# algbio/founderblockgraphs

Measured on AMD Instinct MI355X. Metric: MSA columns segmented/sec, higher is better.
Workload: dtype u32

## Files before the change

founderblockgraphs_amd/csrc/ctx.hip:

```cpp
#include "fbg_internal.h"
#include <chrono>
#include <stdarg.h>
#include <stdio.h>
#include <ctype.h>
#include <string.h>
#include <algorithm>
#include <atomic>
#include <thread>
#include <vector>

static std::string g_global_err;

int fbg_fail(fbg_ctx *ctx, int code, const char *fmt, ...)
{
    char buf[1024];
    va_list ap;
    va_start(ap, fmt);
    vsnprintf(buf, sizeof(buf), fmt, ap);
    va_end(ap);
    if (ctx) ctx->err = buf; else g_global_err = buf;
    return code;
}

int fbg_reserve(fbg_ctx *ctx, DevBuf &b, size_t bytes, std::vector<DevBuf *> *owner, bool accounted)
// ... 166 lines not shown
    {"pure_scan", &FbgOptions::pure_scan},
    {"gapped_rank", &FbgOptions::gapped_rank},
    {"part_tricks_off", &FbgOptions::part_tricks_off},
    {"msd_sample_bins", &FbgOptions::msd_sample_bins},
    {"msd_min_force", &FbgOptions::msd_min_force},
    {"msd_probe", &FbgOptions::msd_probe},
    {"msd_xcd", &FbgOptions::msd_xcd},
    {"rank_no_lean", &FbgOptions::rank_no_lean},
    {"no_stream_upload", &FbgOptions::no_stream_upload},
    {"span_scan", &FbgOptions::span_scan},
    {"span_key_flags", &FbgOptions::span_key_flags},
    {"span_slow_split", &FbgOptions::span_slow_split},
    {"poison", &FbgOptions::poison},
    {"dpw_matrix", &FbgOptions::dpw_matrix},
    {"dp_chain1", &FbgOptions::dp_chain1},
    {"msd_ext", &FbgOptions::msd_ext},
    {"rows_wave", &FbgOptions::rows_wave},
    {"pairs_in_scan", &FbgOptions::pairs_in_scan},
    {"runs_wave_min", &FbgOptions::runs_wave_min},
    {"wave_list_cap", &FbgOptions::wave_list_cap},
    {"cand_local_sort", &FbgOptions::cand_local_sort},
    {"cand_lds_cap", &FbgOptions::cand_lds_cap},
    {"cand_sort_check", &FbgOptions::cand_sort_check},
};

struct InfoKey { const char *name; int64_t (*get)(const fbg_ctx &); };
static const InfoKey g_info_keys[] = {
    {"grs_threshold", [](const fbg_ctx &c) -> int64_t { return c.grs_t; }},
    {"grs_redone", [](const fbg_ctx &c) -> int64_t { return (int64_t)c.grs_redone; }},
    {"dp_kind", [](const fbg_ctx &c) -> int64_t { return c.dp_kind; }},
    {"msd_decline", [](const fbg_ctx &c) -> int64_t { return c.diag.msd_decline; }},
    {"pass1_ahead", [](const fbg_ctx &c) -> int64_t { return c.diag.pass1_ahead; }},
    {"ext_pairs", [](const fbg_ctx &c) -> int64_t { return c.diag.ext_pairs; }},
    {"text_pairs", [](const fbg_ctx &c) -> int64_t { return c.diag.text_pairs; }},
    {"cand_inversions", [](const fbg_ctx &c) -> int64_t { return c.diag.cand_inversions; }},
    {"cand_local_sorted", [](const fbg_ctx &c) -> int64_t { return c.diag.cand_local_sorted; }},
    {"wave_runs", [](const fbg_ctx &c) -> int64_t { return c.diag.wave_runs; }},
    {"rank_lean_used", [](const fbg_ctx &c) -> int64_t { return c.diag.rank_lean_used; }},
    {"rank_lean_launched", [](const fbg_ctx &c) -> int64_t { return c.diag.rank_lean_launched; }},
    {"pairs_rb", [](const fbg_ctx &c) -> int64_t { return c.diag.pairs_rb; }},
    {"key_b", [](const fbg_ctx &c) -> int64_t { return c.key_b; }},
    {"key_K", [](const fbg_ctx &c) -> int64_t { return c.key_K; }},
    {"key_packed", [](const fbg_ctx &c) -> int64_t { return c.key_packed; }},
    {"key_compact", [](const fbg_ctx &c) -> int64_t { return c.key_compact; }},
    {"alloc_calls", [](const fbg_ctx &c) -> int64_t { return (int64_t)c.alloc_calls; }},
    {"alloc_us", [](const fbg_ctx &c) -> int64_t { return (int64_t)c.alloc_us; }},
// ... 112 lines not shown

void fbg_ctx_destroy(fbg_ctx *ctx)
{
    if (!ctx) return;
    (void)hipSetDevice(ctx->device);
    (void)hipStreamSynchronize(ctx->stream);
    fbg_release_all(ctx, ctx->bufs);
    fbg_msd_pre_free(ctx);
    if (ctx->up_stream) {
        (void)hipStreamSynchronize(ctx->up_stream);
        for (auto &e : ctx->up_ev) if (e) (void)hipEventDestroy(e);
        (void)hipStreamDestroy(ctx->up_stream);
    }
    for (auto &t : ctx->timers) {
        if (t.start) (void)hipEventDestroy(t.start);
        if (t.stop) (void)hipEventDestroy(t.stop);
    }
    if (ctx->stager.base) {
        for (int i = 0; i < ctx->stager.nslots; i++) (void)hipEventDestroy(ctx->stager.ev[i]);
        delete[] ctx->stager.ev;
        (void)hipStreamDestroy(ctx->stager.stream);
        (void)hipHostFree(ctx->stager.base);
    }
    if (ctx->aux_fork) (void)hipEventDestroy(ctx->aux_fork);
    if (ctx->aux_join) (void)hipEventDestroy(ctx->aux_join);
    if (ctx->aux) (void)hipStreamDestroy(ctx->aux);
    if (ctx->own_stream) (void)hipStreamDestroy(ctx->stream);
    delete ctx;
}

const char *fbg_last_error(const fbg_ctx *ctx) { return ctx ? ctx->err.c_str() : g_global_err.c_str(); }

int fbg_set_stream(fbg_ctx *ctx, void *hip_stream)
{
    if (!ctx) return FBG_ERR_INVALID;
    FBG_HIP_TRY(ctx, hipStreamSynchronize(ctx->stream));
    if (ctx->own_stream) { (void)hipStreamDestroy(ctx->stream); ctx->own_stream = false; }
    if (hip_stream) {
        ctx->stream = (hipStream_t)hip_stream;
    } else {
        FBG_HIP_TRY(ctx, hipStreamCreateWithFlags(&ctx->stream, hipStreamNonBlocking));
        ctx->own_stream = true;
    }
    return FBG_OK;
}

// ... 368 lines not shown
```

founderblockgraphs_amd/csrc/fbg_internal.h:

```cpp
#pragma once
#include <cstring>
#include <cstdlib>
#include <hip/hip_runtime.h>
#include <stdint.h>
#include <string>
#include <vector>
#include "../../include/fbg_hip.h"

#define FBG_WAVE 64

struct DevBuf {
    void *p = nullptr;
    size_t cap = 0;
    bool listed = false;
    template <class T> T *as() const { return reinterpret_cast<T *>(p); }
};

struct Stager {
    void *base = nullptr;
    size_t slot_bytes = 0;
    int nslots = 0;
    hipEvent_t *ev = nullptr;
    hipStream_t stream = nullptr;
};

struct StageTimer {
    hipEvent_t start = nullptr, stop = nullptr;
    bool recorded = false;
    int launches = 0;
};

struct FbgOptions {
    int64_t no_ranked = 0, no_packed = 0, force_wide = 0, full_keys = 0, no_msd_sort = 0, msd_min = -1, bp_min = -1,
            record_scatter = 0, lcp_text = 0, no_aux_stream = 0, rank_no_threshold = 0, dp_literal = 0, dp_wave = 0,
            dp_safe_window = 0, dp_tile = 0, pure_scan = 0, gapped_rank = 0, part_tricks_off = 0, msd_sample_bins = 0, msd_min_force = 0, msd_probe = 0, msd_xcd = -1, rank_no_lean = 0, no_stream_upload = 0,
            span_scan = 0, span_key_flags = 0, span_slow_split = 0, poison = 0, dpw_matrix = 0, dp_chain1 = 0, msd_ext = 1, rows_wave = 0,
            pairs_in_scan = 1, runs_wave_min = 16, wave_list_cap = 0,
            cand_local_sort = 1, cand_lds_cap = 0, cand_sort_check = 0;
};

enum class IndexKind { none, record, ranked, gapped, span };

struct IndexState {
    bool index_valid = false;
    IndexKind kind = IndexKind::none;
    bool ranked() const { return kind == IndexKind::ranked; }
    bool granked() const { return kind == IndexKind::gapped || kind == IndexKind::span; }
    bool spanned() const { return kind == IndexKind::span; }
    uint32_t *sa_ptr = nullptr;
    uint64_t *rk_keys = nullptr;
    int rk_b = 0, rk_key_bits = 0, rk_K = 0;
    int rk_layout = 0, rk_pb = 0;
    bool grs_flagged = false;
    bool sp_key_flags_sorted = false;
    bool msd_ext_valid = false;
    bool lcp_from_keys = false;
    bool grs_ties_done = false;
    uint32_t n_exc = 0;
    bool part_active = false;
    bool gpart = false;
    int part = 0, nparts = 1;
// ... 11 lines not shown
    int cand_local_sorted = -1;
    int rank_lean_launched = 0;
    int rank_lean_used = 0;
    int pairs_rb = -1;
    int sp_decline = 0;
};

struct SortExtras {
    const uint64_t *ebits = nullptr;
    const uint32_t *payload = nullptr;
    bool key_flags = false;
};

struct MsdPlan;
struct fbg_ctx {
    int device = 0;
    FbgOptions opt;
    std::string err;
    hipStream_t stream = nullptr;
    bool own_stream = false;
    hipStream_t aux = nullptr;
    hipEvent_t aux_fork = nullptr, aux_join = nullptr;
    bool aux_pending = false;
    Stager stager;
    StageTimer timers[FBG_STAGE_COUNT];

    const uint8_t *d_msa = nullptr;
    DevBuf msa_own;
    uint64_t m = 0, n = 0;
    int reversed = 0;
    bool gapfree = true;
    bool have_ignore = false;
    uint8_t ignore_tab[256] = {0};
    uint64_t N = 0;
    uint64_t byte_hist[256] = {0};
    bool allow_wide = false;
    uint32_t mp = 0;
    DevBuf text;
    DevBuf pos, tot;
    DevBuf segtab;
    DevBuf colT;
    DevBuf gwin_rows;

    const uint8_t *up_host = nullptr;
    hipStream_t up_stream = nullptr;
    hipEvent_t up_ev[9] = {};
// ... 21 lines not shown
    DevBuf exc_scratch;
    DevBuf exc;
    int grs_tricks_off = 0;
    uint32_t grs_ign_lo = 0, grs_ign_hi = 0;
    DevBuf gwin;
    DevBuf gbits;
    bool pairs_similar = false;
    bool grs_part_failed = false;
    uint32_t grs_t = 1;
    uint64_t grs_redone = 0;
    DevBuf sp_cells;
    DevBuf sp_flagT;
    DevBuf sp_cwin;
    DevBuf sp_tiles, sp_gstart, sp_gcol, sp_gflags, sp_rstart, sp_rid, sp_gplo, sp_gphi, sp_gval, sp_odd, sp_irr, sp_chain, sp_slow, sp_mins;
    uint32_t sp_chain_n = 0, sp_slow_n = 0;
    uint64_t sp_G = 0, sp_R = 0, sp_n_irr = 0, sp_work = 0;
    uint32_t sp_n_odd[4] = {0, 0, 0, 0}, sp_odd_cap = 0;

    DevBuf keysA, keysB, valsA, valsB, grp, flags, list, tie_list, big_groups, tmp, small, scalars;
    DevBuf msd_ext;
    DevBuf wave_list;
    DevBuf kargs;
    alignas(16) unsigned char kargs_host[512];
    DevBuf msd_w, msd_v;
    DevBuf dp_a, dp_b, dp_c, dp_d, dp_e, dp_f, dp_g, dp_h, io_a, io_b, io_c, io_d;
    DevBuf bt_up, bt_dep;
    DevBuf ps_a, ps_b, ps_c, ps_d, ps_e, ps_f, ps_g, ps_h;
};

int fbg_fail(fbg_ctx *ctx, int code, const char *fmt, ...);
#define FBG_HIP_TRY(ctx, expr)                                                              \
    do {                                                                                    \
        hipError_t e_ = (expr);                                                             \
        if (e_ != hipSuccess)                                                               \
            return fbg_fail((ctx), e_ == hipErrorOutOfMemory ? FBG_ERR_OOM : FBG_ERR_HIP,   \
                            "%s failed: %s (%s:%d)", #expr, hipGetErrorString(e_), __FILE__, \
                            __LINE__);                                                      \
    } while (0)
#define FBG_TRY(expr)                \
    do {                             \
        int rc_ = (expr);            \
        if (rc_ != FBG_OK) return rc_; \
    } while (0)

int fbg_reserve(fbg_ctx *ctx, DevBuf &b, size_t bytes, std::vector<DevBuf *> *owner, bool accounted);
inline int fbg_reserve(fbg_ctx *ctx, DevBuf &b, size_t bytes) { return fbg_reserve(ctx, b, bytes, &ctx->bufs, true); }
// ... 97 lines not shown
```

founderblockgraphs_amd/csrc/host/host_selftest.cpp:

```cpp
#include <cstdio>
#include <cstdlib>
#include <string>
#include <vector>
#include "fasta.hpp"
#include "xgfa.hpp"

int main(int argc, char **argv)
{
    if (argc < 6) {
        std::fprintf(stderr, "usage: %s FASTA GAP_LIMIT ELASTIC PATHS OUT.gfa [BOUNDARY ...]\n", argv[0]);
        return 2;
    }
    Msa msa;
    if (!read_msa(argv[1], std::atol(argv[2]), std::atoi(argv[3]) != 0, std::atoi(argv[4]) != 0, msa)) {
        std::fprintf(stderr, "cannot read %s\n", argv[1]);
        return 3;
    }
    std::printf("%llu %llu\n", (unsigned long long)msa.m, (unsigned long long)msa.n);
    if (argc == 6 || msa.m == 0) return 0;
    std::vector<uint64_t> boundaries;
    int first_boundary = 6;
    BlockGraph g;
    bool have_graph = false;
    if (std::string(argv[6]).rfind("GRAPH=", 0) == 0) {
        first_boundary = 7;
        have_graph = true;
        FILE *fh = std::fopen(argv[6] + 6, "rb");
        uint64_t hdr[2];
        if (!fh || std::fread(hdr, 8, 2, fh) != 2) { std::fprintf(stderr, "cannot read %s\n", argv[6] + 6); return 5; }
        const uint64_t nb = hdr[0], m = hdr[1];
        g.node_of.resize(nb * m); g.rep_row.resize(nb * m); g.first_node.resize(nb + 1); g.edge_count.resize(nb); g.edges.resize(nb * m);
// ... 19 lines not shown
```

founderblockgraphs_amd/csrc/rank_scan.hip:

```cpp
#include <algorithm>
#include <cstring>
#include <vector>
#include "fbg_internal.h"
#include "text_cmp.h"
#include <rocprim/rocprim.hpp>

#include "rank_common.h"

#define RS_ITEMS 4
#define RS_THREADS 256
#define RS_CHUNK (RS_THREADS * RS_ITEMS)

template <int L, bool PLAIN> __global__ __launch_bounds__(RS_THREADS) __attribute__((amdgpu_waves_per_eu(7, 8))) void k_rank_scan(RankArgs a)
{
    __shared__ uint64_t skey[RS_CHUNK + 2 * RS_HALO];
    __shared__ uint32_t srem[RS_CHUNK + 2 * RS_HALO];
    __shared__ uint16_t sq[RS_CHUNK];
    __shared__ uint32_t sqn, s_cand_n, s_tie_n;
    const int lane = threadIdx.x & 63;
    const uint64_t nchunks = (a.own_hi - a.own_lo + RS_CHUNK - 1) / RS_CHUNK;
    if (threadIdx.x == 0) { s_cand_n = 0; s_tie_n = 0; }
    uint64_t w[RS_ITEMS + 1];
    uint32_t v[RS_ITEMS + 1];
    const int my_i = RS_HALO + RS_ITEMS * (int)threadIdx.x;
    const int halo_i = (int)threadIdx.x < RS_HALO ? (int)threadIdx.x : RS_CHUNK + (int)threadIdx.x;
    auto fetch = [&](uint64_t c) {
        const uint64_t base = a.own_lo + c * RS_CHUNK;
        const int lo_i = c == 0 ? RS_HALO : 0;
        const int hi_i = (int)min((uint64_t)(RS_CHUNK + 2 * RS_HALO), a.own_hi - base + RS_HALO);
#pragma unroll
// ... 433 lines not shown
            const uint32_t ln = k + 1 < N ? rs_key_lcp(key, kn, b, key_bits) : 0u;
            bin = min(max(lp, ln) + 1, 63u);
        }
    }
    {
        const int lane = threadIdx.x & 63;
        unsigned long long rest = __ballot(bin != 0xffffffffu);
        while (rest) {
            const int l = __ffsll((long long)rest) - 1;
            const uint32_t v = __shfl(bin, l, 64);
            const unsigned long long same = __ballot(bin == v);
            if (lane == l) { if (v == 64) atomicAdd(&sties, (uint32_t)__popcll(same)); else atomicAdd(&sh[v], (uint32_t)__popcll(same)); }
            rest &= ~same;
        }
    }
    __syncthreads();
    if (threadIdx.x < 64 && sh[threadIdx.x]) atomicAdd(&hist[threadIdx.x], sh[threadIdx.x]);
    if (threadIdx.x == 0) {
        atomicAdd(&counters[2], (unsigned long long)sties);
        atomicAdd(&counters[3], (unsigned long long)min((uint64_t)256, N - (uint64_t)blockIdx.x * 1024 * 256));
    }
}

__global__ void k_count_unfilled(const uint32_t *__restrict__ gmax, uint64_t n, uint32_t g_min, int reversed,
                                 unsigned long long *__restrict__ counters)
{
    const uint64_t x = (uint64_t)blockIdx.x * blockDim.x + threadIdx.x;
    const uint64_t rem = reversed ? x + 1 : n - x;
    const bool miss = x < n && rem > 64 && gmax[x] < g_min;
    const unsigned long long mask = __ballot(miss);
    if ((threadIdx.x & 63) == 0 && mask) atomicAdd(&counters[1 + 3], (unsigned long long)__popcll(mask));
}

__global__ void k_cand_compact(const uint32_t *__restrict__ regions, const uint32_t *__restrict__ counts,
                               const uint32_t *__restrict__ offsets, uint32_t region, uint32_t *__restrict__ out)
{
    const uint32_t c = counts[blockIdx.x] < region ? counts[blockIdx.x] : region, o = offsets[blockIdx.x];
    for (uint32_t i = threadIdx.x; i < c; i += blockDim.x) out[o + i] = regions[(size_t)blockIdx.x * region + i];
}

#define RS_CAND_LDS 4096
__global__ __launch_bounds__(256) void k_cand_sort_compact(const uint32_t *__restrict__ regions, const uint32_t *__restrict__ counts,
                                                           const uint32_t *__restrict__ offsets, uint32_t region, uint32_t *__restrict__ out)
{
    __shared__ uint32_t buf[RS_CAND_LDS];
    const uint32_t c = min(min(counts[blockIdx.x], region), (uint32_t)RS_CAND_LDS), o = offsets[blockIdx.x];
    if (c == 0) return;
    uint32_t P = 2;
    while (P < c) P <<= 1;
    for (uint32_t i = threadIdx.x; i < P; i += blockDim.x) buf[i] = i < c ? regions[(size_t)blockIdx.x * region + i] : 0xffffffffu;
    __syncthreads();
    for (uint32_t k = 2; k <= P; k <<= 1)
        for (uint32_t j = k >> 1; j > 0; j >>= 1) {
            for (uint32_t i = threadIdx.x; i < P; i += blockDim.x) {
                const uint32_t l = i ^ j;
                if (l > i) {
                    const uint32_t x = buf[i], y = buf[l];
                    if ((x > y) == ((i & k) == 0)) { buf[i] = y; buf[l] = x; }
                }
            }
            __syncthreads();
        }
    for (uint32_t i = threadIdx.x; i < c; i += blockDim.x) out[o + i] = buf[i];
}

__global__ void k_cand_inversions(const uint32_t *__restrict__ cand, uint64_t T, unsigned long long *__restrict__ count)
{
    const uint64_t t = (uint64_t)blockIdx.x * blockDim.x + threadIdx.x;
    const unsigned long long mask = __ballot(t + 1 < T && cand[t] >= cand[t + 1]);
    if ((threadIdx.x & 63) == 0 && mask) atomicAdd(count, (unsigned long long)__popcll(mask));
}

#define RS_BIG_GROUPS 1024
#define RS_BIG_MEMBERS 8192
template <int L> __global__ void k_tie_groups(RankArgs a, uint64_t T, int by_list)
{
    const uint64_t t = (uint64_t)blockIdx.x * blockDim.x + threadIdx.x;
    if (t >= T) return;
    const uint64_t k0 = by_list ? (uint64_t)a.cand[t] : a.own_lo + t;
    const uint64_t key = rs_key<L>(a, k0);
    if (k0 > a.own_lo && rs_key<L>(a, k0 - 1) == key) return;
    if (k0 + 1 >= a.own_hi || rs_key<L>(a, k0 + 1) != key) return;
    uint32_t s = 1;
    while (k0 + s < a.own_hi && s <= RS_BIG_MEMBERS && rs_key<L>(a, k0 + s) == key) s++;
    if (s > 64) {
        if (s > RS_BIG_MEMBERS) { a.counters[1] = 1; return; }
        const unsigned long long e = atomicAdd(&a.counters[5], 1ull);
        if (e >= RS_BIG_GROUPS) { a.counters[1] = 1; return; }
        a.big[2 * e] = (uint32_t)k0;
        a.big[2 * e + 1] = s;
        return;
    }
    typedef typename PosT<L>::type pos_t;
    pos_t pos[64];
    uint32_t from = (uint32_t)a.K;
    for (uint32_t i = 0; i < s; i++) {
        pos[i] = (pos_t)rs_pos<L>(a, k0 + i);
        if (rs_rem<L>(a, pos[i]) < (uint32_t)a.K) from = 0;
    }
    for (uint32_t i = 1; i < s; i++) {
        const pos_t cur = pos[i];
        uint32_t j = i;
        while (j > 0) {
            const pos_t o = pos[j - 1];
            const uint32_t h = fbg_extend_match(a.T, (uint64_t)o + from, (uint64_t)cur + from, 0);
            if (a.T[(uint64_t)o + from + h] < a.T[(uint64_t)cur + from + h]) break;
            pos[j] = o;
// ... 255 lines not shown
}

static int rs_order_candidates(fbg_ctx *ctx, RankArgs &a, int layout, uint64_t T, bool sorted_already, int *launches)
{
    hipStream_t st = ctx->stream;
    FBG_TRY(fbg_reserve(ctx, ctx->dp_a, T * 4));
    FBG_TRY(fbg_reserve(ctx, ctx->dp_b, T * 4));
    uint32_t *sorted = ctx->dp_a.as<uint32_t>();
    uint32_t *flat = ctx->dp_e.as<uint32_t>();
    if (!sorted_already)
        FBG_TRY(rs_with_tmp(ctx, [&](void *tmp, size_t &bytes) {
            return rocprim::radix_sort_keys(tmp, bytes, flat, sorted, (size_t)T, 0u, 32u, st);
        }));
    if (ctx->opt.cand_sort_check) {
        unsigned long long *d_inv = ctx->scalars.as<unsigned long long>() + 114, inv = 0;
        FBG_HIP_TRY(ctx, hipMemsetAsync(d_inv, 0, sizeof(inv), st));
        hipLaunchKernelGGL(k_cand_inversions, dim3(fbg_blocks(T, 256)), dim3(256), 0, st, sorted, T, d_inv);
        FBG_HIP_TRY(ctx, hipMemcpyAsync(&inv, d_inv, sizeof(inv), hipMemcpyDeviceToHost, st));
        FBG_HIP_TRY(ctx, hipStreamSynchronize(st));
        ctx->diag.cand_inversions = (int64_t)inv;
    }
    a.cand = sorted;
    a.pm = ctx->dp_b.as<uint32_t>();
    RS_LAUNCH(k_tie_groups, layout, dim3(fbg_blocks(T, 64)), dim3(64), st, a, T, 1);
    RS_LAUNCH(k_tie_big, layout, dim3(RS_BIG_GROUPS), dim3(256), st, a, 0);
    *launches += 3;
    return FBG_OK;
}

static int rs_classify(fbg_ctx *ctx, RankArgs &a, int layout, uint64_t *T_out, int *launches)
{
    hipStream_t st = ctx->stream;
    const uint64_t own = a.own_hi - a.own_lo;
    const unsigned rs_blocks = fbg_blocks(own, RS_CHUNK, 256 * 16);
    const uint32_t region = (uint32_t)((own / rs_blocks) / 8 + 256);
    const uint32_t tie_region = (uint32_t)((own / rs_blocks) / 6 + 256);
    FBG_TRY(fbg_reserve(ctx, ctx->list, (size_t)rs_blocks * region * 4));
    FBG_TRY(fbg_reserve(ctx, ctx->tie_list, (size_t)rs_blocks * tie_region * 4));
    FBG_TRY(fbg_reserve(ctx, ctx->big_groups, RS_BIG_GROUPS * 8));
    a.big = ctx->big_groups.as<uint32_t>();
    if (!a.part_mode) FBG_TRY(rs_wave_list(ctx, a));
    FBG_TRY(fbg_reserve(ctx, ctx->dp_c, (size_t)(rs_blocks + 1) * 4));
    FBG_TRY(fbg_reserve(ctx, ctx->dp_d, (size_t)(rs_blocks + 1) * 4));
    FBG_TRY(fbg_reserve(ctx, ctx->dp_f, (size_t)(rs_blocks + 1) * 4));
    FBG_HIP_TRY(ctx, hipMemsetAsync(ctx->dp_c.p, 0, (size_t)(rs_blocks + 1) * 4, st));
    FBG_HIP_TRY(ctx, hipMemsetAsync(ctx->dp_f.p, 0, (size_t)(rs_blocks + 1) * 4, st));
    a.cand = ctx->list.as<uint32_t>();
// ... 16 lines not shown
        a.pair_stats = ctx->scalars.as<unsigned long long>() + 112;
        FBG_HIP_TRY(ctx, hipMemsetAsync(a.pair_stats, 0, 2 * sizeof(unsigned long long), st));
        FBG_TRY(fbg_reserve(ctx, ctx->ps_g, (size_t)rs_blocks * tie_region * 8));
        FBG_TRY(fbg_reserve(ctx, ctx->ps_h, (size_t)rs_blocks * 4));
        a.pairs = ctx->ps_g.as<uint2>(); a.pair_count = ctx->ps_h.as<uint32_t>();
        static_assert(sizeof(RankArgs) <= sizeof(ctx->kargs_host), "room for the scan's arguments");
        FBG_TRY(fbg_reserve(ctx, ctx->kargs, sizeof(RankArgs)));
        memcpy(ctx->kargs_host, &a, sizeof(RankArgs));
        FBG_HIP_TRY(ctx, hipMemcpyAsync(ctx->kargs.p, ctx->kargs_host, sizeof(RankArgs), hipMemcpyHostToDevice, st));
        hipLaunchKernelGGL(k_rank_scan_lean, dim3(rs_blocks), dim3(RL_THREADS), 0, st, (const RankArgs *)ctx->kargs.p, lf);
    }
    else
        RS_LAUNCH_SCAN(layout, a.g_min <= (uint32_t)a.K || a.values_only, dim3(rs_blocks), st, a);
    FBG_TRY(fbg_stage_end(ctx, FBG_STAGE_RANK_KERNEL, 1));
    {
        hipStream_t ts = st;
        if (!ctx->opt.no_aux_stream) { FBG_TRY(rs_fork(ctx)); ts = ctx->aux; }
        if (lean) hipLaunchKernelGGL(k_tie_pairs, dim3(rs_blocks), dim3(256), 0, ts, a);
        RS_LAUNCH(k_tie_simple, layout, dim3(rs_blocks), dim3(256), ts, a);
    }
    *launches += 2;
    const int rc_rest = [&]() -> int {
        uint32_t *d_counts = a.blk_count, *d_offs = ctx->dp_d.as<uint32_t>();
        FBG_TRY(rs_with_tmp(ctx, [&](void *tmp, size_t &bytes) {
            return rocprim::exclusive_scan(tmp, bytes, d_counts, d_offs, 0u, (size_t)(rs_blocks + 1), rocprim::plus<uint32_t>(), st);
        }));
        uint32_t *d_max = reinterpret_cast<uint32_t *>(a.counters + 6);
        FBG_TRY(rs_with_tmp(ctx, [&](void *tmp, size_t &bytes) {
            return rocprim::reduce(tmp, bytes, d_counts, d_max, 0u, (size_t)rs_blocks, rocprim::maximum<uint32_t>(), st);
        }));
        uint32_t tot = 0, mx = 0;
        FBG_HIP_TRY(ctx, hipMemcpyAsync(&tot, d_offs + rs_blocks, 4, hipMemcpyDeviceToHost, st));
        FBG_HIP_TRY(ctx, hipMemcpyAsync(&mx, d_max, 4, hipMemcpyDeviceToHost, st));
        FBG_HIP_TRY(ctx, hipStreamSynchronize(st));
        const uint64_t T = tot;
        *T_out = T;
        if (mx > region) { *T_out = ~0ull; return rs_join(ctx); }
        if (T > 0) {
            const int64_t cap_opt = ctx->opt.cand_lds_cap;
            const uint32_t lds_cap = cap_opt > 0 && cap_opt < RS_CAND_LDS ? (uint32_t)cap_opt : RS_CAND_LDS;
            const bool local = lean && ctx->opt.cand_local_sort && mx <= lds_cap;
            ctx->diag.cand_local_sorted = local ? 1 : 0;
            if (local) {
                FBG_TRY(fbg_reserve(ctx, ctx->dp_a, T * 4));
                hipLaunchKernelGGL(k_cand_sort_compact, dim3(rs_blocks), dim3(256), 0, st, a.cand, d_counts, d_offs, region, ctx->dp_a.as<uint32_t>());
            } else {
                FBG_TRY(fbg_reserve(ctx, ctx->dp_e, T * 4));
                hipLaunchKernelGGL(k_cand_compact, dim3(rs_blocks), dim3(256), 0, st, a.cand, d_counts, d_offs, region, ctx->dp_e.as<uint32_t>());
            }
            FBG_TRY(rs_order_candidates(ctx, a, layout, T, local, launches));
        }
        return FBG_OK;
    }();
    if (rc_rest != FBG_OK) { (void)rs_join(ctx); return rc_rest; }
    return FBG_OK;
}

static int rs_pick_threshold(fbg_ctx *ctx, RankArgs &a, const uint64_t *keys, uint64_t count, const KeyGeom &geom, int *reject,
                             int *launches)
{
    *reject = 0;
    if (count <= (1u << 22)) return FBG_OK;
    hipStream_t st = ctx->stream;
    unsigned long long *cnt = a.counters;
    unsigned int *d_hist = reinterpret_cast<unsigned int *>(cnt + 8);
    FBG_HIP_TRY(ctx, hipMemsetAsync(d_hist, 0, 64 * sizeof(unsigned int), st));
    hipLaunchKernelGGL(k_tie_sample, dim3(fbg_blocks(count, 1024 * 256)), dim3(256), 0, st, keys, a.pb, count, geom.b, geom.key_bits,
                       cnt, d_hist);
    (*launches)++;
    unsigned long long hs[4];
    unsigned int hh[64];
    FBG_HIP_TRY(ctx, hipMemcpyAsync(hs, cnt, sizeof(hs), hipMemcpyDeviceToHost, st));
    FBG_HIP_TRY(ctx, hipMemcpyAsync(hh, d_hist, sizeof(hh), hipMemcpyDeviceToHost, st));
    FBG_HIP_TRY(ctx, hipStreamSynchronize(st));
    if (hs[2] * 4 > hs[3]) { *reject = 1; return FBG_OK; }
    if (!ctx->opt.rank_no_threshold) {
        const double need = 32.0 / (double)ctx->m * (double)hs[3];
        unsigned long long above = 0;
        for (int g = 63; g >= 1; g--) {
            above += hh[g];
            if ((double)above >= need) { a.g_min = (uint32_t)g; break; }
        }
        if ((double)hs[2] / (double)hs[3] * (double)ctx->m >= 32.0) a.g_min = (uint32_t)geom.K + 1;
    }
    return FBG_OK;
}

int fbg_rank_scan_try(fbg_ctx *ctx, uint64_t *keys, uint32_t *vals, const KeyGeom &geom, int *done)
{
    *done = 0;
    const uint64_t N = ctx->N, n = ctx->n;
    const int layout = rs_layout(geom);
    hipStream_t st = ctx->stream;
    FBG_TRY(fbg_stage_begin(ctx, FBG_STAGE_RANKSCAN));
    unsigned long long *cnt = ctx->scalars.as<unsigned long long>() + 32;
    int launches = 0;
    FBG_TRY(fbg_reserve(ctx, ctx->gmax, (n + 1) * 4));
    RankArgs a;
    rs_args_init(ctx, a, keys, vals, N, layout, geom.pb, geom.b, geom.key_bits, geom.K);
    uint64_t T = 0;
    FBG_HIP_TRY(ctx, hipMemsetAsync(cnt, 0, 8 * sizeof(unsigned long long), st));
    FBG_HIP_TRY(ctx, hipMemsetAsync(ctx->gmax.p, 0, (n + 1) * 4, st));
    int reject = 0;
    FBG_TRY(rs_pick_threshold(ctx, a, keys, N, geom, &reject, &launches));
    if (reject) return fbg_stage_end(ctx, FBG_STAGE_RANKSCAN, launches);
    FBG_TRY(rs_classify(ctx, a, layout, &T, &launches));
    if (T == ~0ull) return fbg_stage_end(ctx, FBG_STAGE_RANKSCAN, launches);
    if (T > 0) {
        RS_LAUNCH(k_runs, layout, dim3(fbg_blocks(T, 64)), dim3(64), st, a, T);
        launches++;
        if (a.runs_wave_min) { RS_LAUNCH(k_runs_long, layout, dim3(a.wl_cap), dim3(64), st, a); launches++; }
    }
    FBG_TRY(rs_join(ctx));
    unsigned long long h[8], ps[2] = {0, 0};
    if (a.g_min > 1)
        hipLaunchKernelGGL(k_count_unfilled, dim3(fbg_blocks(n, 256)), dim3(256), 0, st, a.gmax, n, a.g_min, a.reversed, cnt);
    FBG_HIP_TRY(ctx, hipMemcpyAsync(h, cnt, sizeof(h), hipMemcpyDeviceToHost, st));
    if (a.pair_stats) FBG_HIP_TRY(ctx, hipMemcpyAsync(ps, a.pair_stats, sizeof(ps), hipMemcpyDeviceToHost, st));
    FBG_HIP_TRY(ctx, hipStreamSynchronize(st));
    ctx->diag.ext_pairs = (int64_t)ps[0];
    ctx->diag.text_pairs = (int64_t)ps[1];
    ctx->diag.wave_runs = (int64_t)std::min(h[7], (unsigned long long)a.wl_cap);
    launches++;
    if (h[1] != 0) return fbg_stage_end(ctx, FBG_STAGE_RANKSCAN, launches);
// ... 44 lines not shown

static void rs_part_args(fbg_ctx *ctx, RankArgs &a)
{
    rs_args_init(ctx, a, ctx->ix.rk_keys, ctx->ix.sa_ptr, ctx->ix.part_count + 2 * FBG_PART_HALO, ctx->ix.rk_layout, ctx->ix.rk_pb, ctx->ix.rk_b,
                 ctx->ix.rk_key_bits, ctx->ix.rk_K);
    a.own_lo = FBG_PART_HALO; a.own_hi = FBG_PART_HALO + ctx->ix.part_count;
    a.first_part = ctx->ix.part == 0; a.last_part = ctx->ix.part + 1 == ctx->ix.nparts;
    a.part_mode = ctx->ix.nparts > 1;
}

int fbg_rank_part_classify(fbg_ctx *ctx, uint64_t *keys, uint32_t *vals, uint64_t count, const KeyGeom &geom, int pre_ok,
                           uint8_t *d_blob, int *ok)
{
    const uint64_t n = ctx->n;
    hipStream_t st = ctx->stream;
    FBG_TRY(fbg_stage_begin(ctx, FBG_STAGE_RANKSCAN));
    int launches = 0;
    ctx->ix.part_count = count;
    ctx->ix.part_T = 0;
    fbg_remember_slots(ctx, keys, vals, rs_layout(geom), geom);
    const int layout = rs_layout(geom);
    FBG_TRY(fbg_reserve(ctx, ctx->gmax, (n + 1) * 4));
    unsigned long long *cnt = ctx->scalars.as<unsigned long long>() + 32;
    FBG_HIP_TRY(ctx, hipMemsetAsync(cnt, 0, 8 * sizeof(unsigned long long), st));
    FBG_HIP_TRY(ctx, hipMemsetAsync(ctx->gmax.p, 0, (n + 1) * 4, st));
    int good = pre_ok && count >= 2 * FBG_PART_HALO;
    RankArgs a;
    rs_part_args(ctx, a);
    if (good) {
        int reject = 0;
        FBG_TRY(rs_pick_threshold(ctx, a, keys + a.own_lo, count, geom, &reject, &launches));
        if (reject) good = 0;
    }
    ctx->ix.part_gmin = a.g_min;
    if (good) {
        uint64_t T = 0;
        FBG_TRY(rs_classify(ctx, a, layout, &T, &launches));
        FBG_TRY(rs_join(ctx));
        if (T == ~0ull) good = 0;
        else {
            ctx->ix.part_T = T;
            unsigned long long h[2];
            FBG_HIP_TRY(ctx, hipMemcpyAsync(h, cnt, sizeof(h), hipMemcpyDeviceToHost, st));
            FBG_HIP_TRY(ctx, hipStreamSynchronize(st));
            if (h[1] != 0) good = 0;
        }
    }
// ... 73 lines not shown
    RS_LAUNCH_SCAN(ctx->ix.rk_layout, true, dim3(fbg_blocks(ctx->ix.part_count, RS_CHUNK, 256 * 16)), ctx->stream, a);
    FBG_HIP_TRY(ctx, hipGetLastError());
    ctx->ix.part_gmin = 0;
    return fbg_stage_end(ctx, FBG_STAGE_RANKSCAN, 1);
}

int fbg_rank_finish(fbg_ctx *ctx, uint64_t x0, uint64_t x1, int mode, int disable_tricks, uint64_t *d_out)
{
    FinishArgs f;
    f.gmax = ctx->gmax.as<uint32_t>();
    f.n = ctx->n; f.x0 = x0; f.x1 = x1; f.mode = mode; f.disable_tricks = disable_tricks; f.out = d_out;
    hipLaunchKernelGGL(k_rank_finish, dim3(fbg_blocks(x1 - x0, 256)), dim3(256), 0, ctx->stream, f);
    FBG_HIP_TRY(ctx, hipGetLastError());
    return FBG_OK;
}

int fbg_rank_materialize(fbg_ctx *ctx, uint32_t *d_sa, uint32_t *d_isa, uint32_t *d_pl, uint32_t *d_pr)
{
    RankArgs a;
    rs_args_init(ctx, a, ctx->ix.rk_keys, ctx->ix.sa_ptr, ctx->N, ctx->ix.rk_layout, ctx->ix.rk_pb, ctx->ix.rk_b, ctx->ix.rk_key_bits, ctx->ix.rk_K);
    FBG_TRY(fbg_reserve(ctx, ctx->big_groups, RS_BIG_GROUPS * 8));
    a.big = ctx->big_groups.as<uint32_t>();
    FBG_HIP_TRY(ctx, hipMemsetAsync(a.counters + 5, 0, sizeof(unsigned long long), ctx->stream));
    RS_LAUNCH(k_tie_groups, ctx->ix.rk_layout, dim3(fbg_blocks(ctx->N, 256)), dim3(256), ctx->stream, a, ctx->N, 0);
    RS_LAUNCH(k_tie_big, ctx->ix.rk_layout, dim3(RS_BIG_GROUPS), dim3(256), ctx->stream, a, 1);
    RS_LAUNCH(k_rank_materialize, ctx->ix.rk_layout, dim3(fbg_blocks(ctx->N, 256)), dim3(256), ctx->stream, a, d_sa, d_isa, d_pl, d_pr);
    FBG_HIP_TRY(ctx, hipGetLastError());
    return FBG_OK;
}
```

founderblockgraphs_amd/csrc/suffix_sort.hip:

```cpp
#include "fbg_internal.h"
#include "text_cmp.h"
#include <rocprim/rocprim.hpp>
#include <utility>
#include <cmath>

#define SS_THREADS 256

using fbg_sort_config = rocprim::radix_sort_config<
    rocprim::default_config, rocprim::default_config,
    rocprim::radix_sort_onesweep_config<rocprim::kernel_config<512, 32>, rocprim::kernel_config<1024, 8>, 9,
                                        rocprim::block_radix_rank_algorithm::match>>;

#define PK_ITEMS 8
#define FBG_SEP 0x80
struct PackArgs {
    const uint8_t *T;
    uint64_t N;
    const uint8_t *code;
    int b, K, pb;
    uint64_t *keys;
    uint32_t *vals;
    uint64_t lo, hi, cap;
    int nohi;
    unsigned long long *counter;
// ... 592 lines not shown
    size_t bytes = 0;
    hipError_t e = call(nullptr, bytes);
    if (e != hipSuccess) return fbg_fail(ctx, FBG_ERR_HIP, "rocprim size query: %s", hipGetErrorString(e));
    FBG_TRY(ensure_tmp(ctx, bytes));
    size_t have = ctx->tmp.cap;
    e = call(ctx->tmp.p, have);
    if (e != hipSuccess)
        return fbg_fail(ctx, e == hipErrorOutOfMemory ? FBG_ERR_OOM : FBG_ERR_HIP, "rocprim call: %s", hipGetErrorString(e));
    return FBG_OK;
}

int fbg_key_setup(fbg_ctx *ctx, bool compact, KeyGeom *g, int *launches)
{
    const uint64_t N = ctx->N;
    hipStream_t st = ctx->stream;
    uint8_t *d_code = ctx->small.as<uint8_t>() + 2048;
    const uint64_t *hist = ctx->byte_hist;
    if (hist[0] != 1)
        return fbg_fail(ctx, FBG_ERR_INVALID, "the MSA contains a NUL byte; the text needs a unique 0 sentinel");
    int below = 0, real = 0;
    for (int c = 1; c < 256; c++)
        if (hist[c] && c != '#') { real++; if (c < '#') below++; }
    compact = compact && below == 0 && real >= 1 && real < FBG_SEP;
    uint8_t code[256];
    int sigma = 0;
    if (compact) {
        for (int c = 0; c < 256; c++) {
            if (c == 0 || c == '#') { code[c] = FBG_SEP; continue; }
            code[c] = (uint8_t)sigma;
            if (hist[c]) sigma++;
        }
    } else {
        for (int c = 0; c < 256; c++) { code[c] = (uint8_t)sigma; if (hist[c]) sigma++; }
    }
    int b = 1;
    while ((1 << b) < sigma) b++;
    double H = 0;
    for (int c = 1; c < 256; c++)
        if (hist[c] && !(compact && c == '#')) { const double q = (double)hist[c] / (double)N; H -= q * log2(q); }
    if (H < 0.05) H = 0.05;
    int K = (int)ceil((log2((double)N) + 5.0) / H);
    if (ctx->opt.full_keys || K > 64 / b) K = 64 / b;
    {
        const int passes = (K * b + 8) / 9;
        const int Kfill = (9 * passes) / b;
        K = Kfill < 64 / b ? Kfill : 64 / b;
    }
    g->compact = compact; g->packed = false; g->wide = false; g->pb = 0;
    if (N >= (1ull << 32) || (compact && ctx->opt.force_wide)) {
        if (!compact) return fbg_fail(ctx, FBG_ERR_TOO_LARGE, "text length %llu needs >32-bit positions", (unsigned long long)N);
        int pb = 1;
        while ((1ull << (32 + pb)) < N) pb++;
        g->wide = true; g->pb = pb;
        if (K > (64 - pb) / b) K = (64 - pb) / b;
    } else if (compact && !ctx->opt.no_packed) {
        int pb = 1;
        while ((1ull << pb) < N) pb++;
        const int Kroom = (64 - pb) / b;
        const int Kmin = (int)ceil((log2((double)N) + 3.2) / H);
        if (Kroom >= Kmin) { g->packed = true; g->pb = pb; if (K > Kroom) K = Kroom; }
    }
    g->b = b; g->K = K; g->key_bits = K * b; g->d_code = d_code;
    fbg_note_key_geom(ctx, *g);
    FBG_HIP_TRY(ctx, hipMemcpyAsync(d_code, code, 256, hipMemcpyHostToDevice, st));
    FBG_HIP_TRY(ctx, hipStreamSynchronize(st));
    *launches += 1;
    return FBG_OK;
}

static int sort_slots(fbg_ctx *ctx, const KeyGeom &g, bool key_flags, uint64_t count, uint64_t out_offset)
{
    hipStream_t st = ctx->stream;
    uint64_t *ka = ctx->keysA.as<uint64_t>(), *kb = ctx->keysB.as<uint64_t>() + out_offset;
    if (g.packed) {
        unsigned lo = (unsigned)g.pb;
        const unsigned hi = (unsigned)(g.pb + g.key_bits);
        if (hi == 64 && count < (1u << 23)) lo = 0;
        return with_tmp(ctx, [&](void *tmp, size_t &bytes) {
            return rocprim::radix_sort_keys<fbg_sort_config>(tmp, bytes, ka, kb, (size_t)count, lo, hi, st);
        });
    }
    uint32_t *va = ctx->valsA.as<uint32_t>(), *vb = ctx->valsB.as<uint32_t>() + out_offset;
    unsigned lo = g.wide ? (unsigned)g.pb : key_flags ? 2u : 0u;
    const unsigned hi = lo + (unsigned)g.key_bits;
    if (hi == 64 && count < (1u << 23)) lo = 0;
    return with_tmp(ctx, [&](void *tmp, size_t &bytes) {
        return rocprim::radix_sort_pairs<fbg_sort_config>(tmp, bytes, ka, kb, va, vb, (size_t)count, lo, hi, st);
    });
// ... 362 lines not shown
```

Measured before the change: 63.10 million.

## Gallop tie extents, fuse candidate count scan, loop tie sampling, drop sync

Several independent changes land together. Tie-group extent search now gallops then binary-searches instead of scanning linearly. The candidate-count exclusive scan and max reduction become one single-block kernel that reads back into pinned memory. Tie sampling becomes a grid-stride kernel with a prefetched neighbour window and wave-aggregated histogram atomics, and the histogram memset is folded into the counter memset. A host stream sync after the code-table upload is removed by keeping the table in the context, so the async copy's source stays valid. Together these aim to cut launch, sync and memory-probe overhead, at the cost of a single-block scan that may be slow for large block counts.

After: 64.04 million (median of 6 runs). +1.5%, better.

```diff
diff --git a/founderblockgraphs_amd/csrc/ctx.hip b/founderblockgraphs_amd/csrc/ctx.hip
--- a/founderblockgraphs_amd/csrc/ctx.hip
+++ b/founderblockgraphs_amd/csrc/ctx.hip
@@ -212,6 +212,9 @@
     {"cand_local_sort", &FbgOptions::cand_local_sort},
     {"cand_lds_cap", &FbgOptions::cand_lds_cap},
     {"cand_sort_check", &FbgOptions::cand_sort_check},
+    {"tie_gallop", &FbgOptions::tie_gallop},
+    {"cand_counts_fused", &FbgOptions::cand_counts_fused},
+    {"tie_sample_loop", &FbgOptions::tie_sample_loop},
 };
 
 struct InfoKey { const char *name; int64_t (*get)(const fbg_ctx &); };
@@ -370,6 +373,7 @@
         (void)hipStreamDestroy(ctx->stager.stream);
         (void)hipHostFree(ctx->stager.base);
     }
+    if (ctx->pin_pair) (void)hipHostFree(ctx->pin_pair);
     if (ctx->aux_fork) (void)hipEventDestroy(ctx->aux_fork);
     if (ctx->aux_join) (void)hipEventDestroy(ctx->aux_join);
     if (ctx->aux) (void)hipStreamDestroy(ctx->aux);
diff --git a/founderblockgraphs_amd/csrc/fbg_internal.h b/founderblockgraphs_amd/csrc/fbg_internal.h
--- a/founderblockgraphs_amd/csrc/fbg_internal.h
+++ b/founderblockgraphs_amd/csrc/fbg_internal.h
@@ -36,7 +36,8 @@
             dp_safe_window = 0, dp_tile = 0, pure_scan = 0, gapped_rank = 0, part_tricks_off = 0, msd_sample_bins = 0, msd_min_force = 0, msd_probe = 0, msd_xcd = -1, rank_no_lean = 0, no_stream_upload = 0,
             span_scan = 0, span_key_flags = 0, span_slow_split = 0, poison = 0, dpw_matrix = 0, dp_chain1 = 0, msd_ext = 1, rows_wave = 0,
             pairs_in_scan = 1, runs_wave_min = 16, wave_list_cap = 0,
-            cand_local_sort = 1, cand_lds_cap = 0, cand_sort_check = 0;
+            cand_local_sort = 1, cand_lds_cap = 0, cand_sort_check = 0,
+            tie_gallop = 1, cand_counts_fused = 1, tie_sample_loop = 1;
 };
 
 enum class IndexKind { none, record, ranked, gapped, span };
@@ -94,6 +95,7 @@
     hipStream_t aux = nullptr;
     hipEvent_t aux_fork = nullptr, aux_join = nullptr;
     bool aux_pending = false;
+    uint32_t *pin_pair = nullptr;
     Stager stager;
     StageTimer timers[FBG_STAGE_COUNT];
 
@@ -161,6 +163,7 @@
     DevBuf wave_list;
     DevBuf kargs;
     alignas(16) unsigned char kargs_host[512];
+    uint8_t code_host[256];
     DevBuf msd_w, msd_v;
     DevBuf dp_a, dp_b, dp_c, dp_d, dp_e, dp_f, dp_g, dp_h, io_a, io_b, io_c, io_d;
     DevBuf bt_up, bt_dep;
diff --git a/founderblockgraphs_amd/csrc/host/host_selftest.cpp b/founderblockgraphs_amd/csrc/host/host_selftest.cpp
--- a/founderblockgraphs_amd/csrc/host/host_selftest.cpp
+++ b/founderblockgraphs_amd/csrc/host/host_selftest.cpp
@@ -4,9 +4,53 @@
 #include <vector>
 #include "fasta.hpp"
 #include "xgfa.hpp"
+#include "../tie_extent.h"
+
+static int tie_extent_selftest()
+{
+    const uint32_t cap = 8192;
+    std::vector<uint32_t> sizes;
+    for (uint32_t s = 1; s <= 70; s++) sizes.push_back(s);
+    for (uint32_t s = 8191; s <= 8194; s++) sizes.push_back(s);
+    unsigned long long cases = 0;
+    for (const uint32_t s : sizes)
+        for (int where = 0; where < 3; where++) {
+            const uint64_t before = where == 0 ? 0 : 37, after = where == 2 ? 0 : 29;
+            std::vector<uint64_t> keys;
+            for (uint64_t i = 0; i < before; i++) keys.push_back(10 + i / 3);
+            const uint64_t key = 1000;
+            for (uint32_t i = 0; i < s; i++) keys.push_back(key);
+            for (uint64_t i = 0; i < after; i++) keys.push_back(2000 + i / 2);
+            const uint64_t k0 = before;
+            uint64_t reads = 0;
+            auto key_at = [&](uint64_t k) -> uint64_t {
+                reads++;
+                if (k >= keys.size()) { std::fprintf(stderr, "tie_extent: read of slot %llu beyond the array\n", (unsigned long long)k); std::exit(1); }
+                return keys[k];
+            };
+            std::vector<uint64_t> his = {keys.size()};
+            for (uint64_t cut = 0; cut <= 3 && cut < s; cut++) his.push_back(k0 + s - cut);
+            for (const uint64_t hi : his) {
+                uint32_t want = 1;
+                while (k0 + want < hi && want <= cap && keys[k0 + want] == key) want++;
+                reads = 0;
+                const uint32_t got = fbg_tie_extent(k0, hi, cap, key, key_at);
+                const uint64_t most = FBG_TIE_PROBE + 2 * 14;
+                if (got != want || reads > most) {
+                    std::printf("tie_extent differs: size %u position %d hi %llu: got %u, want %u, %llu reads\n", s, where,
+                                (unsigned long long)hi, got, want, (unsigned long long)reads);
+                    return 1;
+                }
+                cases++;
+            }
+        }
+    std::printf("tie_extent ok %llu\n", cases);
+    return 0;
+}
 
 int main(int argc, char **argv)
 {
+    if (argc == 2 && std::string(argv[1]) == "tie-extent") return tie_extent_selftest();
     if (argc < 6) {
         std::fprintf(stderr, "usage: %s FASTA GAP_LIMIT ELASTIC PATHS OUT.gfa [BOUNDARY ...]\n", argv[0]);
         return 2;
diff --git a/founderblockgraphs_amd/csrc/rank_scan.hip b/founderblockgraphs_amd/csrc/rank_scan.hip
--- a/founderblockgraphs_amd/csrc/rank_scan.hip
+++ b/founderblockgraphs_amd/csrc/rank_scan.hip
@@ -6,6 +6,7 @@
 #include <rocprim/rocprim.hpp>
 
 #include "rank_common.h"
+#include "tie_extent.h"
 
 #define RS_ITEMS 4
 #define RS_THREADS 256
@@ -485,6 +486,61 @@
     }
 }
 
+#define RS_SAMPLE_BLOCKS 512
+__global__ __launch_bounds__(256) void k_tie_sample_loop(const uint64_t *__restrict__ keys, int shift, uint64_t N, int b, int key_bits,
+                                                         uint64_t clusters, unsigned long long *__restrict__ counters,
+                                                         unsigned int *__restrict__ hist)
+{
+    __shared__ unsigned int sh[64];
+    __shared__ unsigned int sties;
+    if (threadIdx.x < 64) sh[threadIdx.x] = 0;
+    if (threadIdx.x == 0) sties = 0;
+    __syncthreads();
+    const int lane = threadIdx.x & 63;
+    unsigned long long looked = 0;
+    uint64_t w[3] = {0, 0, 0};
+    auto fetch = [&](uint64_t c) {
+        const uint64_t k = c * 1024 * 256 + threadIdx.x;
+        if (k < N) {
+            w[1] = keys[k];
+            w[0] = k > 0 ? keys[k - 1] : 0ull;
+            w[2] = k + 1 < N ? keys[k + 1] : 0ull;
+        }
+    };
+    if (blockIdx.x < clusters) fetch(blockIdx.x);
+    for (uint64_t c = blockIdx.x; c < clusters; c += gridDim.x) {
+        const uint64_t k = c * 1024 * 256 + threadIdx.x;
+        const uint64_t key = w[1] >> shift;
+        const uint64_t kp = k > 0 ? w[0] >> shift : ~key, kn = k + 1 < N ? w[2] >> shift : ~key;
+        if (c + gridDim.x < clusters) fetch(c + gridDim.x);
+        uint32_t bin = 0xffffffffu;
+        if (k < N) {
+            if (kp == key || kn == key) {
+                bin = 64;
+            } else {
+                const uint32_t lp = k > 0 ? rs_key_lcp(kp, key, b, key_bits) : 0u;
+                const uint32_t ln = k + 1 < N ? rs_key_lcp(key, kn, b, key_bits) : 0u;
+                bin = min(max(lp, ln) + 1, 63u);
+            }
+        }
+        unsigned long long rest = __ballot(bin != 0xffffffffu);
+        while (rest) {
+            const int l = __ffsll((long long)rest) - 1;
+            const uint32_t v = __shfl(bin, l, 64);
+            const unsigned long long same = __ballot(bin == v);
+            if (lane == l) { if (v == 64) atomicAdd(&sties, (uint32_t)__popcll(same)); else atomicAdd(&sh[v], (uint32_t)__popcll(same)); }
+            rest &= ~same;
+        }
+        looked += min((uint64_t)256, N - c * 1024 * 256);
+    }
+    __syncthreads();
+    if (threadIdx.x < 64 && sh[threadIdx.x]) atomicAdd(&hist[threadIdx.x], sh[threadIdx.x]);
+    if (threadIdx.x == 0 && looked) {
+        if (sties) atomicAdd(&counters[2], (unsigned long long)sties);
+        atomicAdd(&counters[3], looked);
+    }
+}
+
 __global__ void k_count_unfilled(const uint32_t *__restrict__ gmax, uint64_t n, uint32_t g_min, int reversed,
                                  unsigned long long *__restrict__ counters)
 {
@@ -527,6 +583,35 @@
     for (uint32_t i = threadIdx.x; i < c; i += blockDim.x) out[o + i] = buf[i];
 }
 
+#define RS_COUNTS_THREADS 1024
+__global__ __launch_bounds__(RS_COUNTS_THREADS) void k_cand_counts(const uint32_t *__restrict__ counts, uint32_t nb, uint32_t *__restrict__ offs,
+                                                                   uint32_t *__restrict__ tot_max)
+{
+    __shared__ uint32_t wsum[RS_COUNTS_THREADS / 64], wmax[RS_COUNTS_THREADS / 64];
+    const uint32_t lane = threadIdx.x & 63, wv = threadIdx.x >> 6;
+    const uint32_t per = (nb + RS_COUNTS_THREADS - 1) / RS_COUNTS_THREADS;
+    const uint32_t i0 = min(threadIdx.x * per, nb), i1 = min(i0 + per, nb);
+    uint32_t sum = 0, mx = 0;
+    for (uint32_t i = i0; i < i1; i++) { const uint32_t c = counts[i]; sum += c; mx = max(mx, c); }
+    uint32_t inc = sum;
+    for (int d = 1; d < 64; d <<= 1) {
+        const uint32_t o = __shfl_up(inc, d, 64);
+        if (lane >= (uint32_t)d) inc += o;
+    }
+    for (int d = 32; d > 0; d >>= 1) mx = max(mx, (uint32_t)__shfl_xor(mx, d, 64));
+    if (lane == 63) wsum[wv] = inc;
+    if (lane == 0) wmax[wv] = mx;
+    __syncthreads();
+    uint32_t before = inc - sum, total = 0, largest = 0;
+    for (uint32_t v = 0; v < RS_COUNTS_THREADS / 64; v++) {
+        if (v < wv) before += wsum[v];
+        total += wsum[v];
+        largest = max(largest, wmax[v]);
+    }
+    for (uint32_t i = i0; i < i1; i++) { offs[i] = before; before += counts[i]; }
+    if (threadIdx.x == 0) { offs[nb] = total; tot_max[0] = total; tot_max[1] = largest; }
+}
+
 __global__ void k_cand_inversions(const uint32_t *__restrict__ cand, uint64_t T, unsigned long long *__restrict__ count)
 {
     const uint64_t t = (uint64_t)blockIdx.x * blockDim.x + threadIdx.x;
@@ -536,7 +621,7 @@
 
 #define RS_BIG_GROUPS 1024
 #define RS_BIG_MEMBERS 8192
-template <int L> __global__ void k_tie_groups(RankArgs a, uint64_t T, int by_list)
+template <int L> __global__ void k_tie_groups(RankArgs a, uint64_t T, int by_list, int gallop)
 {
     const uint64_t t = (uint64_t)blockIdx.x * blockDim.x + threadIdx.x;
     if (t >= T) return;
@@ -545,7 +630,8 @@
     if (k0 > a.own_lo && rs_key<L>(a, k0 - 1) == key) return;
     if (k0 + 1 >= a.own_hi || rs_key<L>(a, k0 + 1) != key) return;
     uint32_t s = 1;
-    while (k0 + s < a.own_hi && s <= RS_BIG_MEMBERS && rs_key<L>(a, k0 + s) == key) s++;
+    if (gallop) s = fbg_tie_extent(k0, a.own_hi, RS_BIG_MEMBERS, key, [&](uint64_t k) { return rs_key<L>(a, k); });
+    else while (k0 + s < a.own_hi && s <= RS_BIG_MEMBERS && rs_key<L>(a, k0 + s) == key) s++;
     if (s > 64) {
         if (s > RS_BIG_MEMBERS) { a.counters[1] = 1; return; }
         const unsigned long long e = atomicAdd(&a.counters[5], 1ull);
@@ -847,7 +933,7 @@
     }
     a.cand = sorted;
     a.pm = ctx->dp_b.as<uint32_t>();
-    RS_LAUNCH(k_tie_groups, layout, dim3(fbg_blocks(T, 64)), dim3(64), st, a, T, 1);
+    RS_LAUNCH(k_tie_groups, layout, dim3(fbg_blocks(T, 64)), dim3(64), st, a, T, 1, ctx->opt.tie_gallop != 0 ? 1 : 0);
     RS_LAUNCH(k_tie_big, layout, dim3(RS_BIG_GROUPS), dim3(256), st, a, 0);
     *launches += 3;
     return FBG_OK;
@@ -910,17 +996,25 @@
     *launches += 2;
     const int rc_rest = [&]() -> int {
         uint32_t *d_counts = a.blk_count, *d_offs = ctx->dp_d.as<uint32_t>();
-        FBG_TRY(rs_with_tmp(ctx, [&](void *tmp, size_t &bytes) {
-            return rocprim::exclusive_scan(tmp, bytes, d_counts, d_offs, 0u, (size_t)(rs_blocks + 1), rocprim::plus<uint32_t>(), st);
-        }));
         uint32_t *d_max = reinterpret_cast<uint32_t *>(a.counters + 6);
-        FBG_TRY(rs_with_tmp(ctx, [&](void *tmp, size_t &bytes) {
-            return rocprim::reduce(tmp, bytes, d_counts, d_max, 0u, (size_t)rs_blocks, rocprim::maximum<uint32_t>(), st);
-        }));
         uint32_t tot = 0, mx = 0;
-        FBG_HIP_TRY(ctx, hipMemcpyAsync(&tot, d_offs + rs_blocks, 4, hipMemcpyDeviceToHost, st));
-        FBG_HIP_TRY(ctx, hipMemcpyAsync(&mx, d_max, 4, hipMemcpyDeviceToHost, st));
-        FBG_HIP_TRY(ctx, hipStreamSynchronize(st));
+        if (ctx->opt.cand_counts_fused) {
+            if (!ctx->pin_pair) FBG_HIP_TRY(ctx, hipHostMalloc(reinterpret_cast<void **>(&ctx->pin_pair), 2 * sizeof(uint32_t), hipHostMallocDefault));
+            hipLaunchKernelGGL(k_cand_counts, dim3(1), dim3(RS_COUNTS_THREADS), 0, st, d_counts, (uint32_t)rs_blocks, d_offs, d_max);
+            FBG_HIP_TRY(ctx, hipMemcpyAsync(ctx->pin_pair, d_max, 2 * sizeof(uint32_t), hipMemcpyDeviceToHost, st));
+            FBG_HIP_TRY(ctx, hipStreamSynchronize(st));
+            tot = ctx->pin_pair[0]; mx = ctx->pin_pair[1];
+        } else {
+            FBG_TRY(rs_with_tmp(ctx, [&](void *tmp, size_t &bytes) {
+                return rocprim::exclusive_scan(tmp, bytes, d_counts, d_offs, 0u, (size_t)(rs_blocks + 1), rocprim::plus<uint32_t>(), st);
+            }));
+            FBG_TRY(rs_with_tmp(ctx, [&](void *tmp, size_t &bytes) {
+                return rocprim::reduce(tmp, bytes, d_counts, d_max, 0u, (size_t)rs_blocks, rocprim::maximum<uint32_t>(), st);
+            }));
+            FBG_HIP_TRY(ctx, hipMemcpyAsync(&tot, d_offs + rs_blocks, 4, hipMemcpyDeviceToHost, st));
+            FBG_HIP_TRY(ctx, hipMemcpyAsync(&mx, d_max, 4, hipMemcpyDeviceToHost, st));
+            FBG_HIP_TRY(ctx, hipStreamSynchronize(st));
+        }
         const uint64_t T = tot;
         *T_out = T;
         if (mx > region) { *T_out = ~0ull; return rs_join(ctx); }
@@ -944,6 +1038,13 @@
     return FBG_OK;
 }
 
+static int rs_zero_counters(fbg_ctx *ctx, unsigned long long *cnt, uint64_t count)
+{
+    const size_t bytes = 8 * sizeof(unsigned long long) + (count > (1u << 22) ? 64 * sizeof(unsigned int) : 0);
+    FBG_HIP_TRY(ctx, hipMemsetAsync(cnt, 0, bytes, ctx->stream));
+    return FBG_OK;
+}
+
 static int rs_pick_threshold(fbg_ctx *ctx, RankArgs &a, const uint64_t *keys, uint64_t count, const KeyGeom &geom, int *reject,
                              int *launches)
 {
@@ -952,9 +1053,14 @@
     hipStream_t st = ctx->stream;
     unsigned long long *cnt = a.counters;
     unsigned int *d_hist = reinterpret_cast<unsigned int *>(cnt + 8);
-    FBG_HIP_TRY(ctx, hipMemsetAsync(d_hist, 0, 64 * sizeof(unsigned int), st));
-    hipLaunchKernelGGL(k_tie_sample, dim3(fbg_blocks(count, 1024 * 256)), dim3(256), 0, st, keys, a.pb, count, geom.b, geom.key_bits,
-                       cnt, d_hist);
+    const unsigned clusters = fbg_blocks(count, 1024 * 256);
+    if (ctx->opt.tie_sample_loop > 0) {
+        const unsigned grid = ctx->opt.tie_sample_loop == 1 ? RS_SAMPLE_BLOCKS : (unsigned)std::min<int64_t>(ctx->opt.tie_sample_loop, 4096);
+        hipLaunchKernelGGL(k_tie_sample_loop, dim3(std::min(clusters, grid)), dim3(256), 0, st, keys, a.pb, count, geom.b, geom.key_bits,
+                           (uint64_t)clusters, cnt, d_hist);
+    }
+    else
+        hipLaunchKernelGGL(k_tie_sample, dim3(clusters), dim3(256), 0, st, keys, a.pb, count, geom.b, geom.key_bits, cnt, d_hist);
     (*launches)++;
     unsigned long long hs[4];
     unsigned int hh[64];
@@ -987,7 +1093,7 @@
     RankArgs a;
     rs_args_init(ctx, a, keys, vals, N, layout, geom.pb, geom.b, geom.key_bits, geom.K);
     uint64_t T = 0;
-    FBG_HIP_TRY(ctx, hipMemsetAsync(cnt, 0, 8 * sizeof(unsigned long long), st));
+    FBG_TRY(rs_zero_counters(ctx, cnt, N));
     FBG_HIP_TRY(ctx, hipMemsetAsync(ctx->gmax.p, 0, (n + 1) * 4, st));
     int reject = 0;
     FBG_TRY(rs_pick_threshold(ctx, a, keys, N, geom, &reject, &launches));
@@ -1078,7 +1184,7 @@
     const int layout = rs_layout(geom);
     FBG_TRY(fbg_reserve(ctx, ctx->gmax, (n + 1) * 4));
     unsigned long long *cnt = ctx->scalars.as<unsigned long long>() + 32;
-    FBG_HIP_TRY(ctx, hipMemsetAsync(cnt, 0, 8 * sizeof(unsigned long long), st));
+    FBG_TRY(rs_zero_counters(ctx, cnt, count));
     FBG_HIP_TRY(ctx, hipMemsetAsync(ctx->gmax.p, 0, (n + 1) * 4, st));
     int good = pre_ok && count >= 2 * FBG_PART_HALO;
     RankArgs a;
@@ -1198,7 +1304,7 @@
     FBG_TRY(fbg_reserve(ctx, ctx->big_groups, RS_BIG_GROUPS * 8));
     a.big = ctx->big_groups.as<uint32_t>();
     FBG_HIP_TRY(ctx, hipMemsetAsync(a.counters + 5, 0, sizeof(unsigned long long), ctx->stream));
-    RS_LAUNCH(k_tie_groups, ctx->ix.rk_layout, dim3(fbg_blocks(ctx->N, 256)), dim3(256), ctx->stream, a, ctx->N, 0);
+    RS_LAUNCH(k_tie_groups, ctx->ix.rk_layout, dim3(fbg_blocks(ctx->N, 256)), dim3(256), ctx->stream, a, ctx->N, 0, ctx->opt.tie_gallop != 0 ? 1 : 0);
     RS_LAUNCH(k_tie_big, ctx->ix.rk_layout, dim3(RS_BIG_GROUPS), dim3(256), ctx->stream, a, 1);
     RS_LAUNCH(k_rank_materialize, ctx->ix.rk_layout, dim3(fbg_blocks(ctx->N, 256)), dim3(256), ctx->stream, a, d_sa, d_isa, d_pl, d_pr);
     FBG_HIP_TRY(ctx, hipGetLastError());
diff --git a/founderblockgraphs_amd/csrc/suffix_sort.hip b/founderblockgraphs_amd/csrc/suffix_sort.hip
--- a/founderblockgraphs_amd/csrc/suffix_sort.hip
+++ b/founderblockgraphs_amd/csrc/suffix_sort.hip
@@ -638,7 +638,7 @@
     for (int c = 1; c < 256; c++)
         if (hist[c] && c != '#') { real++; if (c < '#') below++; }
     compact = compact && below == 0 && real >= 1 && real < FBG_SEP;
-    uint8_t code[256];
+    uint8_t *code = ctx->code_host;
     int sigma = 0;
     if (compact) {
         for (int c = 0; c < 256; c++) {
@@ -679,7 +679,6 @@
     g->b = b; g->K = K; g->key_bits = K * b; g->d_code = d_code;
     fbg_note_key_geom(ctx, *g);
     FBG_HIP_TRY(ctx, hipMemcpyAsync(d_code, code, 256, hipMemcpyHostToDevice, st));
-    FBG_HIP_TRY(ctx, hipStreamSynchronize(st));
     *launches += 1;
     return FBG_OK;
 }
diff --git a/founderblockgraphs_amd/csrc/tie_extent.h b/founderblockgraphs_amd/csrc/tie_extent.h
--- /dev/null
+++ b/founderblockgraphs_amd/csrc/tie_extent.h
@@ -0,0 +1,35 @@
+#pragma once
+#include <stdint.h>
+
+#if defined(__HIPCC__)
+#define FBG_TIE_HD __host__ __device__
+#else
+#define FBG_TIE_HD
+#endif
+
+#define FBG_TIE_PROBE 8
+
+template <class KeyAt> FBG_TIE_HD inline uint32_t fbg_tie_extent(uint64_t k0, uint64_t hi, uint32_t cap, uint64_t key, KeyAt key_at)
+{
+    const uint64_t room = hi - k0;
+    const uint32_t limit = room < (uint64_t)cap + 1 ? (uint32_t)room : cap + 1;
+    uint32_t lo = 1;
+    while (lo < limit && lo < FBG_TIE_PROBE) {
+        if (key_at(k0 + lo) != key) return lo;
+        lo++;
+    }
+    if (lo >= limit) return limit;
+    uint32_t end = limit;
+    for (uint32_t step = FBG_TIE_PROBE;; step <<= 1) {
+        const uint32_t probe = limit - lo > step ? lo + step - 1 : limit - 1;
+        if (key_at(k0 + probe) != key) { end = probe; break; }
+        lo = probe + 1;
+        if (lo >= limit) return limit;
+    }
+    while (lo < end) {
+        const uint32_t mid = lo + (end - lo) / 2;
+        if (key_at(k0 + mid) == key) lo = mid + 1;
+        else end = mid;
+    }
+    return lo;
+}
```
